# pyani-plus/pyani-plus

Measured on AMD Instinct MI355X. Metric: pairwise genome comparisons/sec (N x N ANI matrix), higher is better.
Workload: dtype u64

## Files before the change

### pyani_plus_amd/csrc/kmer_hash.hip

```cpp
#include <cstdlib>
#include <type_traits>
#include <utility>

#include "pa_internal.h"
#include "murmur_dev.h"

namespace {

using namespace pa_dev;

constexpr int kThreads = 256;
constexpr uint32_t kStageCap = 1024;
constexpr uint32_t kStageCapSecond = 512;

constexpr int pow2_floor(int k) { int c = 1; while (2 * c <= k) c *= 2; return c; }

__device__ __forceinline__ uint32_t find_genome(const uint32_t *__restrict__ genome_blk, uint32_t n, uint32_t blk) {
  uint32_t lo = 0, hi = n;
  while (hi - lo > 1) {
    uint32_t mid = (lo + hi) >> 1;
    if (genome_blk[mid] <= blk) lo = mid; else hi = mid;
  }
  return lo;
}
// ... 26 lines not shown
    region_append(s, find_genome(s.genome_blk, s.n_genomes, t), h);
  } else {
    const unsigned long long g = atomicAdd(reinterpret_cast<unsigned long long *>(s.count), 1ULL);
    if (g < s.cap) {
      s.cand_hash[g] = h;
      s.cand_genome[g] = find_genome(s.genome_blk, s.n_genomes, t);
    }
  }
}

template <uint32_t Cap>
__device__ __forceinline__ void flush_staged(const CandSink &s, const uint64_t (&s_hash)[Cap], const uint32_t (&s_blk)[Cap],
                                             const uint32_t &s_n, unsigned long long &s_base, uint32_t blk0, uint32_t n_blocks64) {
  const uint32_t tid = threadIdx.x;
  __syncthreads();
  const uint32_t n = min(s_n, Cap);
  if (n == 0) return;
  if (s.region_off) {
    const uint32_t b0 = blk0 + blockIdx.x * kThreads;
    const uint32_t b1 = min(b0 + (uint32_t)kThreads, n_blocks64) - 1u;
    const uint32_t g0 = find_genome(s.genome_blk, s.n_genomes, b0);
    if (s.genome_blk[g0 + 1] > b1) {
      if (tid == 0) s_base = atomicAdd(&s.cursor[g0], n);
      __syncthreads();
      const uint64_t room = s.region_off[g0 + 1] - s.region_off[g0];
      uint64_t *__restrict__ dst = s.cand_hash + s.region_off[g0];
      for (uint32_t i = tid; i < n; i += kThreads) {
        const uint64_t slot = s_base + i;
        if (slot < room) dst[slot] = s_hash[i]; else *s.overflow = 1u;
      }
    } else {
      for (uint32_t i = tid; i < n; i += kThreads)
        region_append(s, find_genome(s.genome_blk, s.n_genomes, s_blk[i]), s_hash[i]);
    }
    return;
  }
  if (tid == 0) s_base = atomicAdd(reinterpret_cast<unsigned long long *>(s.count), (unsigned long long)n);
  __syncthreads();
  const unsigned long long base = s_base;
  for (uint32_t i = tid; i < n; i += kThreads) {
    const unsigned long long g = base + i;
    if (g < s.cap) {
      s.cand_hash[g] = s_hash[i];
      s.cand_genome[g] = find_genome(s.genome_blk, s.n_genomes, s_blk[i]);
    }
  }
}

__device__ __forceinline__ uint32_t rev_groups32(uint32_t x) {
  x = __builtin_bitreverse32(x);
  return ((x >> 1) & 0x55555555u) | ((x & 0x55555555u) << 1);
}

enum WordForm { kArithmetic = 0, kFirstTables = 1, kSecondTables = 2 };
template <int K, WordForm FORM>
__global__ __launch_bounds__(kThreads) void kmer_hash_kernel(
    const uint4 *__restrict__ packed, const uint2 *__restrict__ mask, const uint64_t *__restrict__ dirty, uint32_t n_blocks64,
    const uint32_t *__restrict__ genome_blk, uint32_t n_genomes, uint64_t max_hash,
    uint64_t *__restrict__ cand_hash, uint32_t *__restrict__ cand_genome, uint64_t cap,
    unsigned long long *__restrict__ count, const uint64_t *__restrict__ region_off, uint32_t *__restrict__ cursor,
    uint32_t *__restrict__ overflow, uint32_t blk0) {
  static_assert(K >= 1 && K <= 32, "a k-mer is one 64-bit register pair");
  constexpr uint32_t kCap = FORM == kSecondTables ? kStageCapSecond : kStageCap;
  __shared__ uint64_t s_hash[kCap];
  __shared__ uint32_t s_blk[kCap];
  __shared__ uint32_t s_n;
  __shared__ unsigned long long s_base;
  constexpr int kWords = (K + 7) / 8;
  __shared__ uint64_t s_lo[FORM == kFirstTables ? kWords : 1][256];
  __shared__ uint4 s_w[FORM == kSecondTables ? kWords : 1][256];
  __shared__ uint32_t s_hi[FORM != kArithmetic ? kWords : 1][256];

  const uint32_t tid = threadIdx.x;
  const CandSink sink{cand_hash, cand_genome, cap, reinterpret_cast<uint64_t *>(count), region_off, cursor, overflow, genome_blk, n_genomes};
  const uint32_t max_hi = (uint32_t)(max_hash >> 32);
  const bool take_all = max_hi == 0xffffffffu;
  const uint32_t screen_hi = max_hi + 1u;
  if (tid == 0) s_n = 0;
  if constexpr (FORM == kFirstTables) fill_first_products(s_lo, s_hi, tid, std::integral_constant<int, K>{});
  if constexpr (FORM == kSecondTables) fill_second_products(s_w, s_hi, tid, K);
  __syncthreads();

  const uint32_t t = blk0 + blockIdx.x * kThreads + tid;
  if (t < n_blocks64) {
    const uint4 cur = packed[t];
    uint2 pw = make_uint2(0u, 0u);
    if (t > 0) pw = reinterpret_cast<const uint2 *>(packed)[2 * (uint64_t)t - 1];
    uint32_t d1 = 0u, d2 = 0u;
    const uint32_t wave_blk = __builtin_amdgcn_readfirstlane(t & ~63u);
    const uint64_t dirty_word = dirty[wave_blk >> 6];
    if ((dirty_word >> (t & 63u)) & 1ull) {
      const uint2 m = mask[t];
      uint32_t d0 = t > 0 ? mask[t - 1].y : 0xffffffffu;
      d1 = m.x;
      d2 = m.y;
      int c = 1;
#pragma unroll
      for (; 2 * c <= K; c *= 2) {
        d2 |= alignbit(d2, d1, 32 - c);
        d1 |= alignbit(d1, d0, 32 - c);
        d0 |= d0 << c;
      }
      constexpr int cc = pow2_floor(K);
      constexpr int r = K - cc;
      if constexpr (r > 0) {
        d2 |= alignbit(d2, d1, 32 - r);
        d1 |= alignbit(d1, d0, 32 - r);
      }
    }
    const uint32_t bad[2] = {d1, d2};
    if ((d1 & d2) != 0xffffffffu) {
      constexpr uint64_t kMask = (K == 32) ? ~0ULL : ((1ULL << (2 * K)) - 1);
      constexpr uint32_t kMaskHi = (uint32_t)(kMask >> 32);
      uint32_t fw[8] = {pw.x, pw.y, cur.x, cur.y, cur.z, cur.w, 0u, 0u};
      uint32_t rw[6];
#pragma unroll
      for (int j = 0; j < 6; ++j) rw[j] = ~rev_groups32(fw[5 - j]);
      auto columns = [&](auto base_tag, int i_begin, int i_end) {
        constexpr int kBase = decltype(base_tag)::value;
#pragma unroll 1
        for (int i = i_begin; i < i_end; ++i) {
          constexpr int kOff = 33 - K;
          const uint32_t fo = 2u * (uint32_t)((i + kOff) & 15), ro = 30u - 2u * (uint32_t)i;
          uint32_t A[5], B[5];
#pragma unroll
          for (int j = 0; j < 5; ++j) {
            A[j] = alignbit(fw[kBase + j + 1], fw[kBase + j], fo);
            B[j] = alignbit(rw[j + 1], rw[j], ro);
          }
#pragma unroll
          for (int wi = 0; wi < 4; ++wi) {
            const uint32_t f_lo = A[wi], f_hi = A[wi + 1], r_lo = B[3 - wi], r_hi = B[4 - wi];
          const uint64_t f_lsb = u64_of(f_lo, f_hi) & kMask, r_lsb = u64_of(r_lo, r_hi) & kMask;
          const uint64_t fwd = __builtin_amdgcn_uicmpl(f_lsb, r_lsb, 37 );
          uint32_t clo, chi;
          asm("s_nop 1\n\tv_cndmask_b32_e64 %0, %1, %2, %3" : "=v"(clo) : "v"((uint32_t)r_lsb), "v"((uint32_t)f_lsb), "s"(fwd));
          asm("v_cndmask_b32_e64 %0, %1, %2, %3" : "=v"(chi) : "v"((uint32_t)(r_lsb >> 32)), "v"((uint32_t)(f_lsb >> 32)), "s"(fwd), "v"(clo));
          uint64_t P[4] = {0, 0, 0, 0};
#pragma unroll
          for (int j = 0; j < kWords; ++j) {
            const uint32_t src = j < 2 ? clo : chi;
            if constexpr (FORM == kSecondTables) {
              P[j] = second_product(s_w, s_hi, j, src);
            } else if constexpr (FORM == kFirstTables) {
              P[j] = first_product(s_lo, s_hi, j, src);
            } else {
              const uint32_t glo = (src >> (16 * (j & 1))) & 0xffu, ghi = (src >> (16 * (j & 1) + 8)) & 0xffu;
              const uint64_t word = u64_of(ascii_group(glo, K - 8 * j), ascii_group(ghi, K - 8 * j - 4));
              P[j] = word * ((j & 1) ? kC2 : kC1);
            }
          }
          (void)kMaskHi;
          uint64_t U, V;
          if constexpr (FORM == kSecondTables) murmur3_pre_last_mul_of_seconds<K>(P, U, V); else murmur3_pre_last_mul<K>(P, U, V);
          if (passes_screen(U, V, take_all, screen_hi)) {
            const uint64_t h = last_mul_and_fold(U, V);
            if (h > max_hash || ((bad[wi >> 1] >> (16 * (wi & 1) + i)) & 1u)) continue;
            stage_candidate(sink, s_hash, s_blk, s_n, t, h);
          }
          }
        }
      };
      constexpr int kOff0 = 33 - K, kSplit = (kOff0 & 15) ? 16 - (kOff0 & 15) : 16;
      columns(std::integral_constant<int, (kOff0 >> 4)>{}, 0, kSplit);
      if constexpr (kSplit < 16) columns(std::integral_constant<int, (kOff0 >> 4) + 1>{}, kSplit, 16);
    }
  }
  flush_staged(sink, s_hash, s_blk, s_n, s_base, blk0, n_blocks64);
}

template <int K>
__global__ __launch_bounds__(kThreads) void kmer_hash_wide_kernel(
    const uint4 *__restrict__ packed, const uint2 *__restrict__ mask, const uint64_t *__restrict__ dirty, uint32_t n_blocks64,
    const uint32_t *__restrict__ genome_blk, uint32_t n_genomes, uint64_t max_hash,
    uint64_t *__restrict__ cand_hash, uint32_t *__restrict__ cand_genome, uint64_t cap,
    unsigned long long *__restrict__ count, const uint64_t *__restrict__ region_off, uint32_t *__restrict__ cursor,
    uint32_t *__restrict__ overflow, uint32_t blk0) {
  static_assert(K >= 33 && K <= 64, "k-mers of 65 to 128 bits");
  __shared__ uint64_t s_hash[kStageCap];
  __shared__ uint32_t s_blk[kStageCap];
  __shared__ uint32_t s_n;
  __shared__ unsigned long long s_base;
  constexpr int kWords = (K + 7) / 8;
  __shared__ uint64_t s_lo[kWords][256];
  __shared__ uint32_t s_hi[kWords][256];
  const uint32_t tid = threadIdx.x;
  const CandSink sink{cand_hash, cand_genome, cap, reinterpret_cast<uint64_t *>(count), region_off, cursor, overflow, genome_blk, n_genomes};
  const uint32_t max_hi = (uint32_t)(max_hash >> 32);
  const bool take_all = max_hi == 0xffffffffu;
  const uint32_t screen_hi = max_hi + 1u;
  if (tid == 0) s_n = 0;
  fill_first_products(s_lo, s_hi, tid, std::integral_constant<int, K>{});
  __syncthreads();

  const uint32_t t = blk0 + blockIdx.x * kThreads + tid;
  if (t < n_blocks64) {
    const uint4 cur = packed[t];
    const uint4 prev = t > 0 ? packed[t - 1] : make_uint4(0u, 0u, 0u, 0u);
    uint32_t d2 = 0u, d3 = 0u;
    const uint32_t wave_blk = __builtin_amdgcn_readfirstlane(t & ~63u);
    const uint64_t dirty_word = dirty[wave_blk >> 6];
    const uint64_t before = wave_blk ? dirty[(wave_blk >> 6) - 1] >> 63 : 1ull;
    const uint64_t dirty_or_prev = dirty_word | (dirty_word << 1) | before;
    if ((dirty_or_prev >> (t & 63u)) & 1ull) {
      const uint2 m = mask[t];
      uint32_t d0 = 0xffffffffu, d1 = 0xffffffffu;
      if (t > 0) { const uint2 mp = mask[t - 1]; d0 = mp.x; d1 = mp.y; }
      d2 = m.x;
// ... 88 lines not shown
  const uint64_t wg_first = pos0 + ((uint64_t)blockIdx.y * gridDim.x + blockIdx.x) * (uint64_t)(kThreads * kLongIter);
#pragma unroll 1
  for (int it = 0; it < kLongIter; ++it) {
  const uint64_t e = wg_first + (uint64_t)it * kThreads + tid;
  if (e >= pos1 || e + 1 < k) continue;
  const uint64_t a = e + 1 - k;
  {
    const uint64_t m0 = a >> 5, m_last = e >> 5;
    const uint32_t sm = (uint32_t)(a & 31u);
    const uint32_t w0 = mask[m0], w1 = m0 + 1 <= m_last ? mask[m0 + 1] : 0u, w2 = m0 + 2 <= m_last ? mask[m0 + 2] : 0u;
    const uint32_t b0 = alignbit(w1, w0, sm), b1 = alignbit(w2, w1, sm);
    const uint32_t top = k == 64 ? 0xffffffffu : ((1u << (k - 32u)) - 1u);
    if (b0 | (b1 & top)) continue;
  }
  uint32_t F[4], R[4];
  {
    const uint64_t p0 = a >> 4, p_last = e >> 4;
    const uint32_t sp = 2u * (uint32_t)(a & 15u);
    uint32_t w[5];
#pragma unroll
    for (int i = 0; i < 5; ++i) w[i] = p0 + i <= p_last ? packed[p0 + i] : 0u;
#pragma unroll
    for (int i = 0; i < 4; ++i) F[i] = alignbit(w[i + 1], w[i], sp);
    const uint32_t used = 2u * k - 64u;
    if (used < 32u) { F[2] &= (1u << used) - 1u; F[3] = 0u; }
    else if (used < 64u) F[3] &= (1u << (used - 32u)) - 1u;
    const uint32_t C[6] = {~rev_groups32(F[3]), ~rev_groups32(F[2]), ~rev_groups32(F[1]), ~rev_groups32(F[0]), 0u, 0u};
    const uint32_t s = 128u - 2u * k, ws = s >> 5, bs = s & 31u;
#pragma unroll
    for (int i = 0; i < 4; ++i) R[i] = ws ? alignbit(C[i + 2], C[i + 1], bs) : alignbit(C[i + 1], C[i], bs);
    if (used < 32u) { R[2] &= (1u << used) - 1u; R[3] = 0u; }
    else if (used < 64u) R[3] &= (1u << (used - 32u)) - 1u;
  }
  const uint64_t f_hi = u64_of(F[2], F[3]), f_lo = u64_of(F[0], F[1]), r_hi = u64_of(R[2], R[3]), r_lo = u64_of(R[0], R[1]);
  const bool fwd = f_hi < r_hi || (f_hi == r_hi && f_lo <= r_lo);
  uint32_t c[4];
#pragma unroll
  for (int i = 0; i < 4; ++i) c[i] = fwd ? F[i] : R[i];
  uint64_t P[8] = {0, 0, 0, 0, 0, 0, 0, 0};
#pragma unroll
  for (uint32_t j = 0; j < 8; ++j) {
    if (j >= n_words) break;
    P[j] = first_product(s_lo, s_hi, j, c[j >> 1]);
  }
  uint64_t U, V;
  murmur3_pre_last_mul_rt(P, k, U, V);
  if (!passes_screen(U, V, take_all, screen_hi)) continue;
  const uint64_t h = last_mul_and_fold(U, V);
  if (h > max_hash) continue;
  append_candidate(sink, find_genome(genome_blk, n_genomes, (uint32_t)(e >> 6)), h);
  }
}

template <class Kernel>
int launch_blocks(pa_ctx *c, const char *name, Kernel kernel, const KmerHashArgs &a) {
  const ArenaView &v = a.arena;
  const CandSink &s = a.sink;
  return pa_launch(c, name, kernel, false, ceil_div(v.n_blocks64 - a.blk0, kThreads), kThreads, 0, a.stream,
                   reinterpret_cast<const uint4 *>(v.packed), reinterpret_cast<const uint2 *>(v.mask), v.dirty,
                   (uint32_t)v.n_blocks64, s.genome_blk, s.n_genomes, a.max_hash, s.cand_hash, s.cand_genome, s.cap,
                   reinterpret_cast<unsigned long long *>(s.count), s.region_off, s.cursor, s.overflow, (uint32_t)a.blk0);
}

template <int K>
int launch_k(pa_ctx *c, const KmerHashArgs &a) {
  if constexpr (K > 32) {
    return launch_blocks(c, "kmer_hash_wide_kernel", kmer_hash_wide_kernel<K>, a);
  } else {
#ifdef PA_TOOLS
    if constexpr (K == 31) {
      const char *v = PA_TOOL_ENV("PA_KMER_VARIANT");
      if (v && v[0] == '0') return launch_blocks(c, "kmer_hash_kernel<31, kArithmetic>", kmer_hash_kernel<K, kArithmetic>, a);
      if (v && v[0] == '1') return launch_blocks(c, "kmer_hash_kernel<31, kFirstTables>", kmer_hash_kernel<K, kFirstTables>, a);
    }
#endif
    return launch_blocks(c, "kmer_hash_kernel", kmer_hash_kernel<K, kSecondTables>, a);
  }
}

}

int pa_launch_kmer_hash(pa_ctx *c, const KmerHashArgs &a) {
  const uint64_t n_blocks64 = a.arena.n_blocks64;
  PA_REQUIRE(n_blocks64 < (1ULL << 32), "arena too large: %llu blocks of 64 bases", (unsigned long long)n_blocks64);
  if (n_blocks64 <= a.blk0) return PA_OK;
  const char *long_form = PA_TOOL_ENV("PA_KMER_LONG");
  if (a.k > 32 && a.k <= 64 && long_form && long_form[0] == 'p') {
    const CandSink &s = a.sink;
    const uint64_t pos0 = a.blk0 * 64, pos1 = n_blocks64 * 64;
    const uint64_t per_wg = (uint64_t)kThreads * kLongIter;
    const uint64_t n_wg = (pos1 - pos0 + per_wg - 1) / per_wg;
    const uint32_t gx = (uint32_t)std::min<uint64_t>(n_wg, 1u << 20), gy = (uint32_t)((n_wg + gx - 1) / gx);
    PA_REQUIRE(gy <= 65535u, "arena too large for one launch of the long k-mer kernel: %llu positions", (unsigned long long)(pos1 - pos0));
    return PA_LAUNCH_ON(c, a.stream, kmer_hash_long_kernel, LaunchDim(gx, gy), kThreads, 0, a.arena.packed, a.arena.mask, pos0, pos1, a.k,
                        s.genome_blk, s.n_genomes, a.max_hash, s.cand_hash, s.cand_genome, s.cap,
                        reinterpret_cast<unsigned long long *>(s.count), s.region_off, s.cursor, s.overflow);
  }
  PA_REQUIRE((a.blk0 & 63u) == 0, "k-mer hash launch must start at a multiple of 64 blocks, not %llu", (unsigned long long)a.blk0);
  int status = PA_E_INVALID;
  if (!dispatch_value(a.k, value_list<1, 64>{}, [&](auto k) { status = launch_k<k()>(c, a); })) pa_set_error("k=%u outside [1,64]", a.k);
  return status;
}
```

### pyani_plus_amd/csrc/murmur_dev.h

```cpp
#pragma once

#include <hip/hip_runtime.h>

#include <cstdint>

#include "murmur_words.h"

namespace pa_dev {

__device__ __forceinline__ uint32_t alignbit(uint32_t hi, uint32_t lo, uint32_t sh) {
  return __builtin_amdgcn_alignbit(hi, lo, sh);
}

__device__ __forceinline__ uint64_t u64_of(uint32_t lo, uint32_t hi) { return ((uint64_t)hi << 32) | lo; }

__device__ __forceinline__ uint64_t rotl64(uint64_t x, int r) {
  const uint32_t lo = (uint32_t)x, hi = (uint32_t)(x >> 32);
  if (r == 32) return u64_of(hi, lo);
  if (r < 32) return u64_of(alignbit(lo, hi, 32 - r), alignbit(hi, lo, 32 - r));
  return u64_of(alignbit(hi, lo, 64 - r), alignbit(lo, hi, 64 - r));
}

__device__ __forceinline__ uint64_t fmix64(uint64_t k) {
  k ^= k >> 33;
  k *= 0xff51afd7ed558ccdULL;
  k ^= k >> 33;
  k *= 0xc4ceb9fe1a85ec53ULL;
  k ^= k >> 33;
  return k;
}


__device__ __forceinline__ uint64_t times5_plus(uint64_t h, uint64_t c) {
  uint64_t t;
  asm("v_lshl_add_u64 %0, %1, 2, %1" : "=v"(t) : "v"(h));
  return t + c;
}

constexpr uint64_t kF1 = 0xff51afd7ed558ccdULL, kF2 = 0xc4ceb9fe1a85ec53ULL;

template <int K, int N>
__device__ __forceinline__ void murmur3_pre_last_mul(const uint64_t (&P)[N], uint64_t &U, uint64_t &V) {
  static_assert(N >= (K + 7) / 8, "one first product per 8-byte word of the k-mer");
  uint64_t h1 = 42, h2 = 42;
  constexpr int nblocks = K / 16;
  constexpr int tail = K % 16;
#pragma unroll
  for (int i = 0; i < nblocks; ++i) {
    const uint64_t k1 = rotl64(P[2 * i], 31) * kC2;
    h1 ^= k1;
    if (i == 0) {
      h1 = times5_plus(rotl64(h1, 27), 5ULL * 42ULL + 0x52dce729ULL);
    } else {
      h1 = rotl64(h1, 27) + h2;
      h1 = times5_plus(h1, 0x52dce729ULL);
    }
    const uint64_t k2 = rotl64(P[2 * i + 1], 33) * kC1;
    h2 ^= k2;
    h2 = rotl64(h2, 31) + h1;
    h2 = times5_plus(h2, 0x38495ab5ULL);
  }
  if constexpr (tail > 8) h2 ^= rotl64(P[2 * nblocks + 1], 33) * kC1;
  if constexpr (tail > 0) h1 ^= rotl64(P[2 * nblocks], 31) * kC2;
  h1 ^= (uint64_t)K; h2 ^= (uint64_t)K;
  h1 += h2; h2 += h1;
  h1 ^= h1 >> 33; h1 *= kF1; h1 ^= h1 >> 33;
  h2 ^= h2 >> 33; h2 *= kF1; h2 ^= h2 >> 33;
  U = h1;
  V = h2;
}

template <int K, int N>
__device__ __forceinline__ void murmur3_pre_last_mul_of_seconds(const uint64_t (&Kw)[N], uint64_t &U, uint64_t &V) {
  static_assert(N >= (K + 7) / 8, "one second product per 8-byte word of the k-mer");
  uint64_t h1 = 42, h2 = 42;
  constexpr int nblocks = K / 16;
  constexpr int tail = K % 16;
#pragma unroll
  for (int i = 0; i < nblocks; ++i) {
    h1 ^= Kw[2 * i];
    if (i == 0) {
      h1 = times5_plus(rotl64(h1, 27), 5ULL * 42ULL + 0x52dce729ULL);
    } else {
      h1 = rotl64(h1, 27) + h2;
      h1 = times5_plus(h1, 0x52dce729ULL);
    }
    h2 ^= Kw[2 * i + 1];
    uint64_t r2 = rotl64(h2, 31);
    asm("" : "+v"(r2));
    h2 = times5_plus(r2 + h1, 0x38495ab5ULL);
  }
  if constexpr (tail > 8) h2 ^= Kw[2 * nblocks + 1];
  if constexpr (tail > 0) h1 ^= Kw[2 * nblocks];
  h1 ^= (uint64_t)K; h2 ^= (uint64_t)K;
  h1 += h2; h2 += h1;
  h1 ^= h1 >> 33; h1 *= kF1; h1 ^= h1 >> 33;
  h2 ^= h2 >> 33; h2 *= kF1; h2 ^= h2 >> 33;
  U = h1;
  V = h2;
}

__device__ __forceinline__ void murmur3_pre_last_mul_rt(const uint64_t (&P)[8], uint32_t k, uint64_t &U, uint64_t &V) {
  uint64_t h1 = 42, h2 = 42;
  const uint32_t nblocks = k >> 4, tail = k & 15u;
#pragma unroll
  for (uint32_t i = 0; i < 4; ++i) {
    if (i >= nblocks) break;
    h1 ^= rotl64(P[2 * i], 31) * kC2;
    h1 = rotl64(h1, 27) + h2;
    h1 = times5_plus(h1, 0x52dce729ULL);
    h2 ^= rotl64(P[2 * i + 1], 33) * kC1;
    h2 = rotl64(h2, 31) + h1;
    h2 = times5_plus(h2, 0x38495ab5ULL);
  }
  uint64_t t1 = 0, t2 = 0;
#pragma unroll
  for (uint32_t i = 0; i < 4; ++i)
    if (i == nblocks) { t1 = P[2 * i]; t2 = P[2 * i + 1]; }
  if (tail > 8) h2 ^= rotl64(t2, 33) * kC1;
  if (tail > 0) h1 ^= rotl64(t1, 31) * kC2;
  h1 ^= (uint64_t)k;
  h2 ^= (uint64_t)k;
  h1 += h2;
  h2 += h1;
  h1 ^= h1 >> 33; h1 *= kF1; h1 ^= h1 >> 33;
  h2 ^= h2 >> 33; h2 *= kF1; h2 ^= h2 >> 33;
  U = h1;
  V = h2;
}

__device__ __forceinline__ uint32_t last_mul_high_sum_plus1(uint64_t U, uint64_t V) {
  constexpr uint32_t c0 = (uint32_t)kF2, c1 = (uint32_t)(kF2 >> 32);
  const uint32_t u0 = (uint32_t)U, u1 = (uint32_t)(U >> 32), v0 = (uint32_t)V, v1 = (uint32_t)(V >> 32);
  return (__umulhi(u0, c0) + __umulhi(v0, c0) + 1u) + ((u0 + v0) * c1 + (u1 + v1) * c0);
}

__device__ __forceinline__ bool passes_screen(uint64_t U, uint64_t V, bool take_all, uint32_t screen_hi) {
  return take_all || last_mul_high_sum_plus1(U, V) <= screen_hi;
}
__device__ __forceinline__ uint64_t last_mul_and_fold(uint64_t U, uint64_t V) {
  const uint64_t X = U * kF2, Y = V * kF2;
  return (X ^ (X >> 33)) + (Y ^ (Y >> 33));
}

template <int K, int N>
__device__ __forceinline__ uint64_t murmur3_from_products(const uint64_t (&P)[N]) {
  uint64_t U, V;
  murmur3_pre_last_mul<K, N>(P, U, V);
  return last_mul_and_fold(U, V);
}

template <int W, class KInt>
__device__ __forceinline__ void fill_first_products(uint64_t (&s_lo)[W][256], uint32_t (&s_hi)[W][256], uint32_t tid, KInt k_) {
  const int k = (int)k_;
  const int n_words = (int)(((uint32_t)k + 7u) >> 3);
#pragma unroll
  for (int j = 0; j < n_words; ++j) {
    const uint64_t cj = (j & 1) ? kC2 : kC1;
    s_lo[j][tid] = (uint64_t)ascii_group(tid, k - 8 * j) * cj;
    s_hi[j][tid] = (uint32_t)((uint64_t)ascii_group(tid, k - 8 * j - 4) * cj);
  }
}

template <int W>
__device__ __forceinline__ uint64_t first_product(const uint64_t (&s_lo)[W][256], const uint32_t (&s_hi)[W][256], uint32_t j, uint32_t src) {
  const uint32_t glo = (src >> (16u * (j & 1u))) & 0xffu, ghi = (src >> (16u * (j & 1u) + 8u)) & 0xffu;
  const uint64_t lo = s_lo[j][glo];
  return u64_of((uint32_t)lo, (uint32_t)(lo >> 32) + s_hi[j][ghi]);
}

template <int W>
__device__ __forceinline__ void fill_second_products(uint4 (&s_w)[W][256], uint32_t (&s_b)[W][256], uint32_t tid, int k) {
#pragma unroll
  for (int j = 0; j < W; ++j) {
    const WordLoEntry e = word_lo_entry(j, k, tid);
    s_w[j][tid] = make_uint4(e.t_lo, e.t_hi, e.a_hi, e.pad);
    s_b[j][tid] = word_hi_entry(j, k, tid);
  }
}

template <uint32_t SH>
__device__ __forceinline__ uint32_t byte_offset(uint32_t src, uint32_t byte) {
  uint32_t r;
  const uint32_t sh = SH;
  switch (byte) {
    case 0: asm("v_lshlrev_b32_sdwa %0, %1, %2 dst_sel:DWORD dst_unused:UNUSED_PAD src0_sel:DWORD src1_sel:BYTE_0" : "=v"(r) : "v"(sh), "v"(src)); break;
    case 1: asm("v_lshlrev_b32_sdwa %0, %1, %2 dst_sel:DWORD dst_unused:UNUSED_PAD src0_sel:DWORD src1_sel:BYTE_1" : "=v"(r) : "v"(sh), "v"(src)); break;
    case 2: asm("v_lshlrev_b32_sdwa %0, %1, %2 dst_sel:DWORD dst_unused:UNUSED_PAD src0_sel:DWORD src1_sel:BYTE_2" : "=v"(r) : "v"(sh), "v"(src)); break;
    default: asm("v_lshlrev_b32_sdwa %0, %1, %2 dst_sel:DWORD dst_unused:UNUSED_PAD src0_sel:DWORD src1_sel:BYTE_3" : "=v"(r) : "v"(sh), "v"(src)); break;
  }
  return r;
}

template <int W>
__device__ __forceinline__ uint64_t second_product(const uint4 (&s_w)[W][256], const uint32_t (&s_b)[W][256], int j, uint32_t src) {
  const uint32_t off_w = byte_offset<4>(src, 2u * (j & 1)), off_b = byte_offset<2>(src, 2u * (j & 1) + 1u);
  typedef uint32_t u32x4 __attribute__((ext_vector_type(4)));
  u32x4 e = *reinterpret_cast<const u32x4 *>(reinterpret_cast<const char *>(&s_w[j][0]) + off_w);
  asm("" : "+v"(e));
  const uint32_t b = *reinterpret_cast<const uint32_t *>(reinterpret_cast<const char *>(&s_b[j][0]) + off_b);
  return second_product_of(j, e.x, e.y, e.z, b);
}

}
```

### pyani_plus_amd/csrc/murmur_words.h

```cpp
#pragma once

#include <cstdint>

#if defined(__HIPCC__)
#include <hip/hip_runtime.h>
#define PA_WORDS_FN __host__ __device__ __forceinline__
#else
#define PA_WORDS_FN inline
#endif

namespace pa_dev {

constexpr uint64_t kC1 = 0x87c37b91114253d5ULL, kC2 = 0x4cf5ad432745937fULL;

PA_WORDS_FN uint32_t ascii4(uint32_t b8) {
#if defined(__HIP_DEVICE_COMPILE__)
  uint32_t u = (b8 | (b8 << 12)) & 0x000F000Fu;
  uint32_t v = (u | (u << 6)) & 0x03030303u;
  return __builtin_amdgcn_perm(0u, 0x54474341u, v);
#else
  uint32_t a = 0;
  for (int i = 0; i < 4; ++i) a |= ((0x54474341u >> (8 * ((b8 >> (2 * i)) & 3u))) & 0xffu) << (8 * i);
  return a;
#endif
}

PA_WORDS_FN uint32_t ascii_group(uint32_t b8, int nv) {
  const uint32_t a = ascii4(b8);
  return nv >= 4 ? a : (nv <= 0 ? 0u : (a & ((1u << (8 * nv)) - 1u)));
}

PA_WORDS_FN constexpr uint64_t word_c_first(int j) { return (j & 1) ? kC2 : kC1; }
PA_WORDS_FN constexpr uint64_t word_c_second(int j) { return (j & 1) ? kC1 : kC2; }

struct WordLoEntry {
  uint32_t t_lo, t_hi, a_hi, pad;
};

PA_WORDS_FN WordLoEntry word_lo_entry(int j, int k, uint32_t g) {
  const uint64_t a = (uint64_t)ascii_group(g, k - 8 * j) * word_c_first(j);
  const uint32_t a_lo = (uint32_t)a;
  const uint64_t cb = word_c_second(j);
  const uint64_t t = (j & 1) ? (((uint64_t)a_lo << 33) + (a_lo >> 31)) * cb : ((uint64_t)a_lo << 31) * cb;
  return WordLoEntry{(uint32_t)t, (uint32_t)(t >> 32), (uint32_t)(a >> 32), 0u};
}

PA_WORDS_FN uint32_t word_hi_entry(int j, int k, uint32_t g) {
  return (uint32_t)((uint64_t)ascii_group(g, k - 8 * j - 4) * word_c_first(j));
}

PA_WORDS_FN uint64_t second_product_of(int j, uint32_t t_lo, uint32_t t_hi, uint32_t a_hi, uint32_t b) {
  const uint32_t s = a_hi + b;
  const uint64_t t = ((uint64_t)t_hi << 32) | t_lo;
  if (j & 1) {
    const uint64_t c = word_c_second(j) << 1;
    const uint64_t m = (uint64_t)s * (uint32_t)c + t;
    return ((uint64_t)((uint32_t)(m >> 32) + s * (uint32_t)(c >> 32)) << 32) | (uint32_t)m;
  }
  const uint64_t c = word_c_second(j);
  const uint32_t x = s >> 1;
  const uint64_t m = (uint64_t)x * (uint32_t)c + t;
  return ((uint64_t)((uint32_t)(m >> 32) + (x * (uint32_t)(c >> 32) + (s << 31))) << 32) | (uint32_t)m;
}

}
```

### pyani_plus_amd/csrc/pa_internal.h

```cpp
#pragma once

#include <hip/hip_runtime.h>

#include <algorithm>
#include <cstdarg>
#include <cstdint>
#include <cstdio>
#include <cstring>
#include <initializer_list>
#include <string>
#include <type_traits>
#include <vector>

#include "../../include/pyani_hip.h"
#include "pa_launch_geom.h"

void pa_set_error(const char *fmt, ...);

#define PA_HIP(call)                                                                          \
  do {                                                                                        \
    hipError_t _e = (call);                                                                   \
    if (_e != hipSuccess) {                                                                   \
      pa_set_error("%s failed: %s (%s:%d)", #call, hipGetErrorString(_e), __FILE__, __LINE__); \
      return PA_E_HIP;                                                                        \
// ... 63 lines not shown
  void release() {
    if (p) (void)hipFree(p);
    if (budget) budget->held -= bytes;
    p = nullptr;
    bytes = 0;
  }
  template <typename T>
  T *as() const { return reinterpret_cast<T *>(p); }
};

struct ProfPhase {
  double total_ms = 0.0;
  uint64_t launches = 0;
  std::vector<std::pair<hipEvent_t, hipEvent_t>> pending;
};

struct ScalarSlot {
  uint32_t word, words;
  constexpr uint32_t bytes() const { return words * 4u; }
  constexpr bool apart_from(ScalarSlot o) const { return word + words <= o.word || o.word + o.words <= word; }
};
constexpr bool slots_apart(uint32_t region_bytes, std::initializer_list<ScalarSlot> slots) {
  for (const ScalarSlot *a = slots.begin(); a != slots.end(); ++a) {
    if ((a->word + a->words) * 4u > region_bytes || (a->words % 2 == 0 && a->word % 2)) return false;
    for (const ScalarSlot *b = a + 1; b != slots.end(); ++b)
      if (!a->apart_from(*b)) return false;
  }
  return true;
}

constexpr uint32_t kCtxScalarBytes = 128;
constexpr ScalarSlot kCandCount{0, 2};
constexpr ScalarSlot kSketchTotal{2, 2};
constexpr ScalarSlot kDenseIds{4, 4};
constexpr uint32_t kDenseOr = 0, kDenseDistinct = 1;
constexpr ScalarSlot kCompactTotal{8, 2};
constexpr ScalarSlot kRegionOverflow{12, 1};
constexpr ScalarSlot kNjPick{16, 8};
constexpr ScalarSlot kNjBad{24, 4};
static_assert(slots_apart(kCtxScalarBytes, {kCandCount, kSketchTotal, kDenseIds, kCompactTotal, kRegionOverflow, kNjPick, kNjBad}),
              "two slots of pa_ctx::counters overlap or leave the block");

constexpr uint32_t kDictScalarBytes = 64;
constexpr ScalarSlot kDictCounters{0, 2};
constexpr uint32_t kDictIdCounter = 0, kDictSpecialId = 1;
constexpr ScalarSlot kDictPreparedFp{2, 4};
constexpr ScalarSlot kDictTileFp{6, 4};
static_assert(slots_apart(kDictScalarBytes, {kDictCounters, kDictPreparedFp, kDictTileFp}),
              "two slots of pa_ctx::dict_scalars overlap or leave the block");

constexpr uint32_t kPinnedBytes = 64;

#define PA_CTX_BUFFERS(ONE, PAIR)                                                                                   \
  PAIR(cand_keys) PAIR(cand_vals) ONE(genome_blk) ONE(counters) ONE(hist) ONE(flags) ONE(scan_tmp) ONE(region_off) \
  ONE(region_cursor) ONE(dirty) PAIR(dict_keys) PAIR(dict_vals) ONE(ids) ONE(post_genome) ONE(bitrows)             \
  ONE(dict_scalars) ONE(cls_i) ONE(cls_j) ONE(cls_score) ONE(cls_cov) ONE(bin2d) ONE(tetra_tab) ONE(nj_work)

struct pa_ctx {
  int device = 0;
  hipStream_t stream = nullptr;
  bool own_stream = false;
  hipDeviceProp_t prop;
#define PA_ONE(name) DevBuf name;
#define PA_PAIR(name) DevBuf name[2];
  PA_CTX_BUFFERS(PA_ONE, PA_PAIR)
#undef PA_ONE
#undef PA_PAIR
  template <class Fn>
  void each_buffer(Fn &&fn) {
#define PA_ONE(name) fn(name);
#define PA_PAIR(name) fn(name[0]); fn(name[1]);
    PA_CTX_BUFFERS(PA_ONE, PA_PAIR)
#undef PA_ONE
#undef PA_PAIR
  }
  template <typename T = uint32_t>
  T *slot(ScalarSlot s) const { return reinterpret_cast<T *>(counters.as<uint32_t>() + s.word); }
  template <typename T = uint32_t>
  T *dict_slot(ScalarSlot s) const { return reinterpret_cast<T *>(dict_scalars.as<uint32_t>() + s.word); }
  bool dict_prepared = false;
  uint64_t dict_prepared_postings = 0;
  uint32_t dict_prepared_cap = 0;
  hipStream_t copy_stream = nullptr;
  void *frag_work = nullptr;
  uint64_t *h_pinned = nullptr;
  bool prof_on = false;
  ProfPhase prof[PA_PROF_NPHASES];
  std::vector<hipEvent_t> event_pool;
};

class ReadBack {
 public:
  explicit ReadBack(pa_ctx *c) : c_(c) {}
  template <typename T>
  int queue(const T *d_src, T *out, uint32_t count = 1) {
    static_assert(std::is_trivially_copyable<T>::value && alignof(T) <= 8, "ReadBack copies plain scalars");
    const uint64_t bytes = (uint64_t)count * sizeof(T);
    PA_REQUIRE(n_ < kMaxItems && used_ + bytes <= kPinnedBytes, "read-back of %llu bytes behind %u in %u copies exceeds the pinned block of %u bytes",
               (unsigned long long)bytes, used_, n_, kPinnedBytes);
    PA_HIP(hipMemcpyAsync(reinterpret_cast<char *>(c_->h_pinned) + used_, d_src, bytes, hipMemcpyDeviceToHost, c_->stream));
    items_[n_++] = Item{out, used_, (uint32_t)bytes};
    used_ = (used_ + (uint32_t)bytes + 7u) & ~7u;
    return PA_OK;
  }
  int wait() {
    PA_HIP(hipStreamSynchronize(c_->stream));
    for (uint32_t i = 0; i < n_; ++i) memcpy(items_[i].out, reinterpret_cast<const char *>(c_->h_pinned) + items_[i].at, items_[i].bytes);
    n_ = used_ = 0;
    return PA_OK;
  }

 private:
  static constexpr uint32_t kMaxItems = 4;
  struct Item {
    void *out;
    uint32_t at, bytes;
  };
  pa_ctx *c_;
  Item items_[kMaxItems];
  uint32_t n_ = 0, used_ = 0;
};
template <typename T>
int pa_read_back(pa_ctx *c, const T *d_src, T *out, uint32_t count = 1) {
  ReadBack rb(c);
  PA_TRY(rb.queue(d_src, out, count));
  return rb.wait();
}

struct ProfScope {
  pa_ctx *c;
  int phase;
  hipEvent_t e0 = nullptr, e1 = nullptr;
  ProfScope(pa_ctx *ctx, int ph);
  ~ProfScope();
};
// ... 139 lines not shown
```

Before: 81.88 million.

## Precompute k-mer hash lookup tables on host and copy them into shared memory

Each block now copies per-k lookup tables from a device image instead of computing the second-product tables itself. The image is built once per k on the host, cached on the device, and deduplicates words whose table contents match. This shrinks shared memory use, which may raise occupancy, and removes per-block table arithmetic. The candidate screen also switches to a sum-based screen word with a slightly looser bound, which may let a few more candidates reach the exact check.

```diff
diff --git a/pyani_plus_amd/csrc/kmer_hash.hip b/pyani_plus_amd/csrc/kmer_hash.hip
--- a/pyani_plus_amd/csrc/kmer_hash.hip
+++ b/pyani_plus_amd/csrc/kmer_hash.hip
@@ -109,7 +109,7 @@
     const uint32_t *__restrict__ genome_blk, uint32_t n_genomes, uint64_t max_hash,
     uint64_t *__restrict__ cand_hash, uint32_t *__restrict__ cand_genome, uint64_t cap,
     unsigned long long *__restrict__ count, const uint64_t *__restrict__ region_off, uint32_t *__restrict__ cursor,
-    uint32_t *__restrict__ overflow, uint32_t blk0) {
+    uint32_t *__restrict__ overflow, uint32_t blk0, const uint4 *__restrict__ image) {
   static_assert(K >= 1 && K <= 32, "a k-mer is one 64-bit register pair");
   constexpr uint32_t kCap = FORM == kSecondTables ? kStageCapSecond : kStageCap;
   __shared__ uint64_t s_hash[kCap];
@@ -118,17 +118,20 @@
   __shared__ unsigned long long s_base;
   constexpr int kWords = (K + 7) / 8;
   __shared__ uint64_t s_lo[FORM == kFirstTables ? kWords : 1][256];
-  __shared__ uint4 s_w[FORM == kSecondTables ? kWords : 1][256];
-  __shared__ uint32_t s_hi[FORM != kArithmetic ? kWords : 1][256];
+  __shared__ uint32_t s_hi[FORM == kFirstTables ? kWords : 1][256];
+  __shared__ __attribute__((aligned(16))) unsigned char s_img[FORM == kSecondTables ? image_bytes(K) : 16];
 
   const uint32_t tid = threadIdx.x;
   const CandSink sink{cand_hash, cand_genome, cap, reinterpret_cast<uint64_t *>(count), region_off, cursor, overflow, genome_blk, n_genomes};
   const uint32_t max_hi = (uint32_t)(max_hash >> 32);
-  const bool take_all = max_hi == 0xffffffffu;
-  const uint32_t screen_hi = max_hi + 1u;
+  constexpr bool kSumScreen = FORM == kSecondTables;
+  const bool take_all = kSumScreen ? screen_takes_all(max_hi) : max_hi == 0xffffffffu;
+  const uint32_t screen_hi = max_hi + (kSumScreen ? 2u : 1u);
+  uint64_t screen_one_hi = 1ULL << 32;
+  asm("" : "+v"(screen_one_hi));
   if (tid == 0) s_n = 0;
   if constexpr (FORM == kFirstTables) fill_first_products(s_lo, s_hi, tid, std::integral_constant<int, K>{});
-  if constexpr (FORM == kSecondTables) fill_second_products(s_w, s_hi, tid, K);
+  if constexpr (FORM == kSecondTables) copy_image<K>(s_img, image, tid);
   __syncthreads();
 
   const uint32_t t = blk0 + blockIdx.x * kThreads + tid;
@@ -191,7 +194,7 @@
           for (int j = 0; j < kWords; ++j) {
             const uint32_t src = j < 2 ? clo : chi;
             if constexpr (FORM == kSecondTables) {
-              P[j] = second_product(s_w, s_hi, j, src);
+              P[j] = second_product<K>(s_img, j, src);
             } else if constexpr (FORM == kFirstTables) {
               P[j] = first_product(s_lo, s_hi, j, src);
             } else {
@@ -203,7 +206,7 @@
           (void)kMaskHi;
           uint64_t U, V;
           if constexpr (FORM == kSecondTables) murmur3_pre_last_mul_of_seconds<K>(P, U, V); else murmur3_pre_last_mul<K>(P, U, V);
-          if (passes_screen(U, V, take_all, screen_hi)) {
+          if (kSumScreen ? (take_all || screen_word(U, V, screen_one_hi) <= screen_hi) : passes_screen(U, V, take_all, screen_hi)) {
             const uint64_t h = last_mul_and_fold(U, V);
             if (h > max_hash || ((bad[wi >> 1] >> (16 * (wi & 1) + i)) & 1u)) continue;
             stage_candidate(sink, s_hash, s_blk, s_n, t, h);
@@ -398,14 +401,30 @@
   }
 }
 
-template <class Kernel>
-int launch_blocks(pa_ctx *c, const char *name, Kernel kernel, const KmerHashArgs &a) {
+template <class Kernel, class... Extra>
+int launch_blocks(pa_ctx *c, const char *name, Kernel kernel, const KmerHashArgs &a, Extra... extra) {
   const ArenaView &v = a.arena;
   const CandSink &s = a.sink;
   return pa_launch(c, name, kernel, false, ceil_div(v.n_blocks64 - a.blk0, kThreads), kThreads, 0, a.stream,
                    reinterpret_cast<const uint4 *>(v.packed), reinterpret_cast<const uint2 *>(v.mask), v.dirty,
                    (uint32_t)v.n_blocks64, s.genome_blk, s.n_genomes, a.max_hash, s.cand_hash, s.cand_genome, s.cap,
-                   reinterpret_cast<unsigned long long *>(s.count), s.region_off, s.cursor, s.overflow, (uint32_t)a.blk0);
+                   reinterpret_cast<unsigned long long *>(s.count), s.region_off, s.cursor, s.overflow, (uint32_t)a.blk0, extra...);
+}
+
+constexpr uint64_t kImageSlotBytes = (kImageMaxBytes + 255u) & ~255u;
+int image_on_device(pa_ctx *c, uint32_t k, hipStream_t stream, const uint4 **image) {
+  static_assert(sizeof(c->kmer_image_ready) / sizeof(c->kmer_image_ready[0]) == kImageMaxK + 1, "one flag per k");
+  PA_TRY(c->kmer_images.reserve((kImageMaxK + 1) * kImageSlotBytes));
+  unsigned char *slot = c->kmer_images.as<unsigned char>() + k * kImageSlotBytes;
+  if (!c->kmer_image_ready[k]) {
+    std::vector<unsigned char> host(image_bytes((int)k));
+    fill_image((int)k, host.data());
+    PA_HIP(hipMemcpyAsync(slot, host.data(), host.size(), hipMemcpyHostToDevice, stream ? stream : c->stream));
+    PA_HIP(hipStreamSynchronize(stream ? stream : c->stream));
+    c->kmer_image_ready[k] = true;
+  }
+  *image = reinterpret_cast<const uint4 *>(slot);
+  return PA_OK;
 }
 
 template <int K>
@@ -416,11 +435,14 @@
 #ifdef PA_TOOLS
     if constexpr (K == 31) {
       const char *v = PA_TOOL_ENV("PA_KMER_VARIANT");
-      if (v && v[0] == '0') return launch_blocks(c, "kmer_hash_kernel<31, kArithmetic>", kmer_hash_kernel<K, kArithmetic>, a);
-      if (v && v[0] == '1') return launch_blocks(c, "kmer_hash_kernel<31, kFirstTables>", kmer_hash_kernel<K, kFirstTables>, a);
+      const uint4 *none = nullptr;
+      if (v && v[0] == '0') return launch_blocks(c, "kmer_hash_kernel<31, kArithmetic>", kmer_hash_kernel<K, kArithmetic>, a, none);
+      if (v && v[0] == '1') return launch_blocks(c, "kmer_hash_kernel<31, kFirstTables>", kmer_hash_kernel<K, kFirstTables>, a, none);
     }
 #endif
-    return launch_blocks(c, "kmer_hash_kernel", kmer_hash_kernel<K, kSecondTables>, a);
+    const uint4 *image = nullptr;
+    PA_TRY(image_on_device(c, K, a.stream, &image));
+    return launch_blocks(c, "kmer_hash_kernel", kmer_hash_kernel<K, kSecondTables>, a, image);
   }
 }
 
diff --git a/pyani_plus_amd/csrc/murmur_dev.h b/pyani_plus_amd/csrc/murmur_dev.h
--- a/pyani_plus_amd/csrc/murmur_dev.h
+++ b/pyani_plus_amd/csrc/murmur_dev.h
@@ -36,8 +36,6 @@
   asm("v_lshl_add_u64 %0, %1, 2, %1" : "=v"(t) : "v"(h));
   return t + c;
 }
-
-constexpr uint64_t kF1 = 0xff51afd7ed558ccdULL, kF2 = 0xc4ceb9fe1a85ec53ULL;
 
 template <int K, int N>
 __device__ __forceinline__ void murmur3_pre_last_mul(const uint64_t (&P)[N], uint64_t &U, uint64_t &V) {
@@ -169,14 +167,13 @@
   return u64_of((uint32_t)lo, (uint32_t)(lo >> 32) + s_hi[j][ghi]);
 }
 
-template <int W>
-__device__ __forceinline__ void fill_second_products(uint4 (&s_w)[W][256], uint32_t (&s_b)[W][256], uint32_t tid, int k) {
-#pragma unroll
-  for (int j = 0; j < W; ++j) {
-    const WordLoEntry e = word_lo_entry(j, k, tid);
-    s_w[j][tid] = make_uint4(e.t_lo, e.t_hi, e.a_hi, e.pad);
-    s_b[j][tid] = word_hi_entry(j, k, tid);
-  }
+template <int K>
+__device__ __forceinline__ void copy_image(unsigned char *s_img, const uint4 *__restrict__ image, uint32_t tid) {
+  constexpr uint32_t n16 = image_bytes(K) / 16u;
+  uint4 *dst = reinterpret_cast<uint4 *>(s_img);
+#pragma unroll
+  for (uint32_t i = 0; i < n16; i += 256u)
+    if (i + 256u <= n16 || i + tid < n16) dst[i + tid] = image[i + tid];
 }
 
 template <uint32_t SH>
@@ -192,13 +189,14 @@
   return r;
 }
 
-template <int W>
-__device__ __forceinline__ uint64_t second_product(const uint4 (&s_w)[W][256], const uint32_t (&s_b)[W][256], int j, uint32_t src) {
-  const uint32_t off_w = byte_offset<4>(src, 2u * (j & 1)), off_b = byte_offset<2>(src, 2u * (j & 1) + 1u);
+template <int K>
+__device__ __forceinline__ uint64_t second_product(const unsigned char *s_img, int j, uint32_t src) {
+  const uint32_t off_w = byte_offset<4>(src, 2u * (j & 1));
   typedef uint32_t u32x4 __attribute__((ext_vector_type(4)));
-  u32x4 e = *reinterpret_cast<const u32x4 *>(reinterpret_cast<const char *>(&s_w[j][0]) + off_w);
+  u32x4 e = *reinterpret_cast<const u32x4 *>(&s_img[image_lo_offset(j, K)] + off_w);
   asm("" : "+v"(e));
-  const uint32_t b = *reinterpret_cast<const uint32_t *>(reinterpret_cast<const char *>(&s_b[j][0]) + off_b);
+  uint32_t b = 0u;
+  if (image_has_hi(j, K)) b = *reinterpret_cast<const uint32_t *>(&s_img[image_hi_offset(j, K)] + byte_offset<2>(src, 2u * (j & 1) + 1u));
   return second_product_of(j, e.x, e.y, e.z, b);
 }
 
diff --git a/pyani_plus_amd/csrc/murmur_words.h b/pyani_plus_amd/csrc/murmur_words.h
--- a/pyani_plus_amd/csrc/murmur_words.h
+++ b/pyani_plus_amd/csrc/murmur_words.h
@@ -63,4 +63,70 @@
   return ((uint64_t)((uint32_t)(m >> 32) + (x * (uint32_t)(c >> 32) + (s << 31))) << 32) | (uint32_t)m;
 }
 
+
+constexpr uint32_t kImageLoTableBytes = 256u * 16u;
+PA_WORDS_FN constexpr int image_words(int k) { return (k + 7) / 8; }
+PA_WORDS_FN constexpr int word_lo_bases(int j, int k) { return k - 8 * j < 4 ? k - 8 * j : 4; }
+PA_WORDS_FN constexpr int word_hi_bases(int j, int k) { return k - 8 * j - 4 < 0 ? 0 : (k - 8 * j - 4 < 4 ? k - 8 * j - 4 : 4); }
+constexpr uint32_t kImageHiTableBytes = 256u * 4u;
+
+PA_WORDS_FN constexpr int image_lo_class(int j, int k) {
+  for (int i = j & 1; i < j; i += 2)
+    if (word_lo_bases(i, k) == word_lo_bases(j, k)) return i;
+  return j;
 }
+PA_WORDS_FN constexpr int image_hi_class(int j, int k) {
+  for (int i = j & 1; i < j; i += 2)
+    if (word_hi_bases(i, k) == word_hi_bases(j, k)) return i;
+  return j;
+}
+PA_WORDS_FN constexpr bool image_has_hi(int j, int k) { return word_hi_bases(j, k) > 0; }
+
+PA_WORDS_FN constexpr uint32_t image_lo_offset(int j, int k) {
+  uint32_t off = 0;
+  for (int i = 0; i < image_lo_class(j, k); ++i)
+    if (image_lo_class(i, k) == i) off += kImageLoTableBytes;
+  return off;
+}
+PA_WORDS_FN constexpr uint32_t image_lo_bytes(int k) {
+  uint32_t off = 0;
+  for (int i = 0; i < image_words(k); ++i)
+    if (image_lo_class(i, k) == i) off += kImageLoTableBytes;
+  return off;
+}
+PA_WORDS_FN constexpr uint32_t image_hi_offset(int j, int k) {
+  uint32_t off = image_lo_bytes(k);
+  for (int i = 0; i < image_hi_class(j, k); ++i)
+    if (image_has_hi(i, k) && image_hi_class(i, k) == i) off += kImageHiTableBytes;
+  return off;
+}
+PA_WORDS_FN constexpr uint32_t image_bytes(int k) {
+  uint32_t off = image_lo_bytes(k);
+  for (int i = 0; i < image_words(k); ++i)
+    if (image_has_hi(i, k) && image_hi_class(i, k) == i) off += kImageHiTableBytes;
+  return off;
+}
+constexpr int kImageMaxK = 32;
+constexpr uint32_t kImageMaxBytes = 4u * (kImageLoTableBytes + kImageHiTableBytes);
+
+inline void fill_image(int k, unsigned char *out) {
+  for (int j = 0; j < image_words(k); ++j) {
+    if (image_lo_class(j, k) == j) {
+      WordLoEntry *lo = reinterpret_cast<WordLoEntry *>(out + image_lo_offset(j, k));
+      for (uint32_t g = 0; g < 256; ++g) lo[g] = word_lo_entry(j, k, g);
+    }
+    if (image_has_hi(j, k) && image_hi_class(j, k) == j) {
+      uint32_t *hi = reinterpret_cast<uint32_t *>(out + image_hi_offset(j, k));
+      for (uint32_t g = 0; g < 256; ++g) hi[g] = word_hi_entry(j, k, g);
+    }
+  }
+}
+
+constexpr uint64_t kF1 = 0xff51afd7ed558ccdULL, kF2 = 0xc4ceb9fe1a85ec53ULL;
+PA_WORDS_FN constexpr bool screen_takes_all(uint32_t max_hi) { return max_hi >= 0xfffffffeu; }
+PA_WORDS_FN uint32_t screen_word(uint64_t U, uint64_t V, uint64_t one_hi = 1ULL << 32) { return (uint32_t)(((U + V) * kF2 + one_hi) >> 32); }
+PA_WORDS_FN bool passes_sum_screen(uint64_t U, uint64_t V, uint32_t max_hi) {
+  return screen_takes_all(max_hi) || screen_word(U, V) <= max_hi + 2u;
+}
+
+}
diff --git a/pyani_plus_amd/csrc/pa_internal.h b/pyani_plus_amd/csrc/pa_internal.h
--- a/pyani_plus_amd/csrc/pa_internal.h
+++ b/pyani_plus_amd/csrc/pa_internal.h
@@ -139,8 +139,8 @@
 constexpr uint32_t kPinnedBytes = 64;
 
 #define PA_CTX_BUFFERS(ONE, PAIR)                                                                                   \
-  PAIR(cand_keys) PAIR(cand_vals) ONE(genome_blk) ONE(counters) ONE(hist) ONE(flags) ONE(scan_tmp) ONE(region_off) \
-  ONE(region_cursor) ONE(dirty) PAIR(dict_keys) PAIR(dict_vals) ONE(ids) ONE(post_genome) ONE(bitrows)             \
+  PAIR(cand_keys) PAIR(cand_vals) ONE(genome_blk) ONE(kmer_images) ONE(counters) ONE(hist) ONE(flags) ONE(scan_tmp) \
+  ONE(region_off) ONE(region_cursor) ONE(dirty) PAIR(dict_keys) PAIR(dict_vals) ONE(ids) ONE(post_genome) ONE(bitrows) \
   ONE(dict_scalars) ONE(cls_i) ONE(cls_j) ONE(cls_score) ONE(cls_cov) ONE(bin2d) ONE(tetra_tab) ONE(nj_work)
 
 struct pa_ctx {
@@ -168,6 +168,7 @@
   bool dict_prepared = false;
   uint64_t dict_prepared_postings = 0;
   uint32_t dict_prepared_cap = 0;
+  bool kmer_image_ready[33] = {};
   hipStream_t copy_stream = nullptr;
   void *frag_work = nullptr;
   uint64_t *h_pinned = nullptr;
```

Measured after the change: 84.25 million (median of 6 runs). 2.9% higher.

## Share second-product tables by word role and screen candidates on summed product

Applied to the files above, without the earlier changes.

Word tables in shared memory are now keyed by role (parity plus number of valid bases), so words with identical roles share one table slot and empty high groups skip their LDS load. The candidate screen now computes one high-half product of U+V instead of separate products, using a looser bound. The odd-word hi computation uses a fused shift-add instruction. This aims to cut LDS footprint, loads and ALU work in the hot per-k-mer path, at the cost of a looser screen that may let more candidates through to the full hash.

```diff
diff --git a/pyani_plus_amd/csrc/kmer_hash.hip b/pyani_plus_amd/csrc/kmer_hash.hip
--- a/pyani_plus_amd/csrc/kmer_hash.hip
+++ b/pyani_plus_amd/csrc/kmer_hash.hip
@@ -102,7 +102,7 @@
   return ((x >> 1) & 0x55555555u) | ((x & 0x55555555u) << 1);
 }
 
-enum WordForm { kArithmetic = 0, kFirstTables = 1, kSecondTables = 2 };
+enum WordForm { kArithmetic = 0, kFirstTables = 1, kSecondTables = 2, kSecondTablesPerWord = 3 };
 template <int K, WordForm FORM>
 __global__ __launch_bounds__(kThreads) void kmer_hash_kernel(
     const uint4 *__restrict__ packed, const uint2 *__restrict__ mask, const uint64_t *__restrict__ dirty, uint32_t n_blocks64,
@@ -111,24 +111,33 @@
     unsigned long long *__restrict__ count, const uint64_t *__restrict__ region_off, uint32_t *__restrict__ cursor,
     uint32_t *__restrict__ overflow, uint32_t blk0) {
   static_assert(K >= 1 && K <= 32, "a k-mer is one 64-bit register pair");
-  constexpr uint32_t kCap = FORM == kSecondTables ? kStageCapSecond : kStageCap;
+  constexpr bool kSeconds = FORM == kSecondTables || FORM == kSecondTablesPerWord;
+  constexpr bool kByRole = FORM == kSecondTables;
+  constexpr bool kSumScreen = FORM == kSecondTables;
+  constexpr bool kShiftAdd = FORM == kSecondTables;
+  using Tab = SecondTables<K, kByRole>;
+  constexpr uint32_t kCap = kSeconds ? kStageCapSecond : kStageCap;
   __shared__ uint64_t s_hash[kCap];
   __shared__ uint32_t s_blk[kCap];
   __shared__ uint32_t s_n;
   __shared__ unsigned long long s_base;
   constexpr int kWords = (K + 7) / 8;
   __shared__ uint64_t s_lo[FORM == kFirstTables ? kWords : 1][256];
-  __shared__ uint4 s_w[FORM == kSecondTables ? kWords : 1][256];
-  __shared__ uint32_t s_hi[FORM != kArithmetic ? kWords : 1][256];
+  __shared__ uint4 s_w[kSeconds ? Tab::kLoSlots : 1][256];
+  __shared__ uint32_t s_hi[kSeconds ? (Tab::kHiSlots > 0 ? Tab::kHiSlots : 1) : FORM == kFirstTables ? kWords : 1][256];
 
   const uint32_t tid = threadIdx.x;
   const CandSink sink{cand_hash, cand_genome, cap, reinterpret_cast<uint64_t *>(count), region_off, cursor, overflow, genome_blk, n_genomes};
   const uint32_t max_hi = (uint32_t)(max_hash >> 32);
   const bool take_all = max_hi == 0xffffffffu;
   const uint32_t screen_hi = max_hi + 1u;
+  const bool take_all_sum = screen_takes_all(max_hash);
+  const uint32_t screen_bound = screen_bound_of(max_hash);
+  uint64_t two32 = kTwo32;
+  if constexpr (FORM == kSecondTables) asm volatile("" : "+v"(two32));
   if (tid == 0) s_n = 0;
   if constexpr (FORM == kFirstTables) fill_first_products(s_lo, s_hi, tid, std::integral_constant<int, K>{});
-  if constexpr (FORM == kSecondTables) fill_second_products(s_w, s_hi, tid, K);
+  if constexpr (kSeconds) fill_second_products<K, kByRole>(s_w, s_hi, tid);
   __syncthreads();
 
   const uint32_t t = blk0 + blockIdx.x * kThreads + tid;
@@ -190,8 +199,8 @@
 #pragma unroll
           for (int j = 0; j < kWords; ++j) {
             const uint32_t src = j < 2 ? clo : chi;
-            if constexpr (FORM == kSecondTables) {
-              P[j] = second_product(s_w, s_hi, j, src);
+            if constexpr (kSeconds) {
+              P[j] = second_product<K, kByRole, kShiftAdd>(s_w, s_hi, j, src);
             } else if constexpr (FORM == kFirstTables) {
               P[j] = first_product(s_lo, s_hi, j, src);
             } else {
@@ -202,8 +211,8 @@
           }
           (void)kMaskHi;
           uint64_t U, V;
-          if constexpr (FORM == kSecondTables) murmur3_pre_last_mul_of_seconds<K>(P, U, V); else murmur3_pre_last_mul<K>(P, U, V);
-          if (passes_screen(U, V, take_all, screen_hi)) {
+          if constexpr (kSeconds) murmur3_pre_last_mul_of_seconds<K>(P, U, V); else murmur3_pre_last_mul<K>(P, U, V);
+          if (kSumScreen ? passes_screen_sum(U, V, take_all_sum, screen_bound, two32) : passes_screen(U, V, take_all, screen_hi)) {
             const uint64_t h = last_mul_and_fold(U, V);
             if (h > max_hash || ((bad[wi >> 1] >> (16 * (wi & 1) + i)) & 1u)) continue;
             stage_candidate(sink, s_hash, s_blk, s_n, t, h);
@@ -418,6 +427,7 @@
       const char *v = PA_TOOL_ENV("PA_KMER_VARIANT");
       if (v && v[0] == '0') return launch_blocks(c, "kmer_hash_kernel<31, kArithmetic>", kmer_hash_kernel<K, kArithmetic>, a);
       if (v && v[0] == '1') return launch_blocks(c, "kmer_hash_kernel<31, kFirstTables>", kmer_hash_kernel<K, kFirstTables>, a);
+      if (v && v[0] == '2') return launch_blocks(c, "kmer_hash_kernel<31, kSecondTablesPerWord>", kmer_hash_kernel<K, kSecondTablesPerWord>, a);
     }
 #endif
     return launch_blocks(c, "kmer_hash_kernel", kmer_hash_kernel<K, kSecondTables>, a);
diff --git a/pyani_plus_amd/csrc/murmur_dev.h b/pyani_plus_amd/csrc/murmur_dev.h
--- a/pyani_plus_amd/csrc/murmur_dev.h
+++ b/pyani_plus_amd/csrc/murmur_dev.h
@@ -36,8 +36,6 @@
   asm("v_lshl_add_u64 %0, %1, 2, %1" : "=v"(t) : "v"(h));
   return t + c;
 }
-
-constexpr uint64_t kF1 = 0xff51afd7ed558ccdULL, kF2 = 0xc4ceb9fe1a85ec53ULL;
 
 template <int K, int N>
 __device__ __forceinline__ void murmur3_pre_last_mul(const uint64_t (&P)[N], uint64_t &U, uint64_t &V) {
@@ -138,10 +136,6 @@
 __device__ __forceinline__ bool passes_screen(uint64_t U, uint64_t V, bool take_all, uint32_t screen_hi) {
   return take_all || last_mul_high_sum_plus1(U, V) <= screen_hi;
 }
-__device__ __forceinline__ uint64_t last_mul_and_fold(uint64_t U, uint64_t V) {
-  const uint64_t X = U * kF2, Y = V * kF2;
-  return (X ^ (X >> 33)) + (Y ^ (Y >> 33));
-}
 
 template <int K, int N>
 __device__ __forceinline__ uint64_t murmur3_from_products(const uint64_t (&P)[N]) {
@@ -169,13 +163,26 @@
   return u64_of((uint32_t)lo, (uint32_t)(lo >> 32) + s_hi[j][ghi]);
 }
 
-template <int W>
-__device__ __forceinline__ void fill_second_products(uint4 (&s_w)[W][256], uint32_t (&s_b)[W][256], uint32_t tid, int k) {
-#pragma unroll
-  for (int j = 0; j < W; ++j) {
-    const WordLoEntry e = word_lo_entry(j, k, tid);
-    s_w[j][tid] = make_uint4(e.t_lo, e.t_hi, e.a_hi, e.pad);
-    s_b[j][tid] = word_hi_entry(j, k, tid);
+template <int K, bool BY_ROLE>
+struct SecondTables {
+  static constexpr int kWords = word_count(K);
+  static constexpr int kLoSlots = BY_ROLE ? word_slot_count(K, false) : kWords;
+  static constexpr int kHiSlots = BY_ROLE ? word_slot_count(K, true) : kWords;
+  static constexpr bool fills(int j, bool hi) { return BY_ROLE ? word_fills_slot(j, K, hi) : true; }
+  static constexpr int slot(int j, bool hi) { return BY_ROLE ? word_slot(j, K, hi) : j; }
+};
+
+template <int K, bool BY_ROLE, int NW, int NB>
+__device__ __forceinline__ void fill_second_products(uint4 (&s_w)[NW][256], uint32_t (&s_b)[NB][256], uint32_t tid) {
+  using Tab = SecondTables<K, BY_ROLE>;
+  static_assert(NW >= Tab::kLoSlots && NB >= Tab::kHiSlots, "one table per slot");
+#pragma unroll
+  for (int j = 0; j < Tab::kWords; ++j) {
+    if (Tab::fills(j, false)) {
+      const WordLoEntry e = word_lo_entry(j, K, tid);
+      s_w[Tab::slot(j, false)][tid] = make_uint4(e.t_lo, e.t_hi, e.a_hi, e.pad);
+    }
+    if (Tab::fills(j, true)) s_b[Tab::slot(j, true)][tid] = word_hi_entry(j, K, tid);
   }
 }
 
@@ -192,14 +199,19 @@
   return r;
 }
 
-template <int W>
-__device__ __forceinline__ uint64_t second_product(const uint4 (&s_w)[W][256], const uint32_t (&s_b)[W][256], int j, uint32_t src) {
-  const uint32_t off_w = byte_offset<4>(src, 2u * (j & 1)), off_b = byte_offset<2>(src, 2u * (j & 1) + 1u);
+template <int K, bool BY_ROLE, bool SHIFT_ADD, int NW, int NB>
+__device__ __forceinline__ uint64_t second_product(const uint4 (&s_w)[NW][256], const uint32_t (&s_b)[NB][256], int j, uint32_t src) {
+  using Tab = SecondTables<K, BY_ROLE>;
+  const uint32_t off_w = byte_offset<4>(src, 2u * (j & 1));
   typedef uint32_t u32x4 __attribute__((ext_vector_type(4)));
-  u32x4 e = *reinterpret_cast<const u32x4 *>(reinterpret_cast<const char *>(&s_w[j][0]) + off_w);
+  u32x4 e = *reinterpret_cast<const u32x4 *>(reinterpret_cast<const char *>(&s_w[Tab::slot(j, false)][0]) + off_w);
   asm("" : "+v"(e));
-  const uint32_t b = *reinterpret_cast<const uint32_t *>(reinterpret_cast<const char *>(&s_b[j][0]) + off_b);
-  return second_product_of(j, e.x, e.y, e.z, b);
-}
-
-}
+  uint32_t b = 0u;
+  if (Tab::slot(j, true) >= 0) {
+    const uint32_t off_b = byte_offset<2>(src, 2u * (j & 1) + 1u);
+    b = *reinterpret_cast<const uint32_t *>(reinterpret_cast<const char *>(&s_b[Tab::slot(j, true)][0]) + off_b);
+  }
+  return second_product_of(j, e.x, e.y, e.z, b, SHIFT_ADD);
+}
+
+}
diff --git a/pyani_plus_amd/csrc/murmur_words.h b/pyani_plus_amd/csrc/murmur_words.h
--- a/pyani_plus_amd/csrc/murmur_words.h
+++ b/pyani_plus_amd/csrc/murmur_words.h
@@ -49,7 +49,7 @@
   return (uint32_t)((uint64_t)ascii_group(g, k - 8 * j - 4) * word_c_first(j));
 }
 
-PA_WORDS_FN uint64_t second_product_of(int j, uint32_t t_lo, uint32_t t_hi, uint32_t a_hi, uint32_t b) {
+PA_WORDS_FN uint64_t second_product_of(int j, uint32_t t_lo, uint32_t t_hi, uint32_t a_hi, uint32_t b, bool shift_add = false) {
   const uint32_t s = a_hi + b;
   const uint64_t t = ((uint64_t)t_hi << 32) | t_lo;
   if (j & 1) {
@@ -60,7 +60,67 @@
   const uint64_t c = word_c_second(j);
   const uint32_t x = s >> 1;
   const uint64_t m = (uint64_t)x * (uint32_t)c + t;
+#if defined(__HIP_DEVICE_COMPILE__)
+  if (shift_add) {
+    uint32_t hi;
+    asm("v_lshl_add_u32 %0, %1, 31, %2" : "=v"(hi) : "v"(s), "v"((uint32_t)(m >> 32)));
+    return ((uint64_t)(hi + x * (uint32_t)(c >> 32)) << 32) | (uint32_t)m;
+  }
+#endif
+  (void)shift_add;
   return ((uint64_t)((uint32_t)(m >> 32) + (x * (uint32_t)(c >> 32) + (s << 31))) << 32) | (uint32_t)m;
 }
 
+PA_WORDS_FN constexpr int word_count(int k) { return (k + 7) / 8; }
+PA_WORDS_FN constexpr int group_role(int parity, int n_valid) {
+  return n_valid <= 0 ? 0 : 1 + 4 * parity + ((n_valid < 4 ? n_valid : 4) - 1);
 }
+PA_WORDS_FN constexpr int word_lo_role(int j, int k) { return group_role(j & 1, k - 8 * j); }
+PA_WORDS_FN constexpr int word_hi_role(int j, int k) { return group_role(j & 1, k - 8 * j - 4); }
+PA_WORDS_FN constexpr int word_role(int j, int k, bool hi) { return hi ? word_hi_role(j, k) : word_lo_role(j, k); }
+
+PA_WORDS_FN constexpr bool word_fills_slot(int j, int k, bool hi) {
+  if (word_role(j, k, hi) == 0) return false;
+  for (int i = 0; i < j; ++i)
+    if (word_role(i, k, hi) == word_role(j, k, hi)) return false;
+  return true;
+}
+PA_WORDS_FN constexpr int word_slot(int j, int k, bool hi) {
+  if (word_role(j, k, hi) == 0) return -1;
+  int first = j;
+  for (int i = j - 1; i >= 0; --i)
+    if (word_role(i, k, hi) == word_role(j, k, hi)) first = i;
+  int slot = 0;
+  for (int i = 0; i < first; ++i) slot += word_fills_slot(i, k, hi) ? 1 : 0;
+  return slot;
+}
+PA_WORDS_FN constexpr int word_slot_count(int k, bool hi) {
+  int n = 0;
+  for (int j = 0; j < word_count(k); ++j) n += word_fills_slot(j, k, hi) ? 1 : 0;
+  return n;
+}
+
+constexpr uint64_t kF1 = 0xff51afd7ed558ccdULL, kF2 = 0xc4ceb9fe1a85ec53ULL;
+
+PA_WORDS_FN constexpr bool screen_takes_all(uint64_t max_hash) { return (uint32_t)(max_hash >> 32) >= 0xfffffffeu; }
+PA_WORDS_FN constexpr uint32_t screen_bound_of(uint64_t max_hash) { return (uint32_t)(max_hash >> 32) + 2u; }
+
+constexpr uint64_t kTwo32 = 1ULL << 32;
+PA_WORDS_FN uint32_t sum_product_high_plus1(uint64_t U, uint64_t V, uint64_t two32 = kTwo32) {
+  constexpr uint32_t c0 = (uint32_t)kF2, c1 = (uint32_t)(kF2 >> 32);
+  const uint64_t W = U + V;
+  const uint32_t w0 = (uint32_t)W, w1 = (uint32_t)(W >> 32);
+  const uint64_t m = (uint64_t)w0 * c0 + two32;
+  return (uint32_t)(m >> 32) + (w0 * c1 + w1 * c0);
+}
+
+PA_WORDS_FN bool passes_screen_sum(uint64_t U, uint64_t V, bool take_all, uint32_t screen_bound, uint64_t two32 = kTwo32) {
+  return take_all || sum_product_high_plus1(U, V, two32) <= screen_bound;
+}
+
+PA_WORDS_FN uint64_t last_mul_and_fold(uint64_t U, uint64_t V) {
+  const uint64_t X = U * kF2, Y = V * kF2;
+  return (X ^ (X >> 33)) + (Y ^ (Y >> 33));
+}
+
+}
```

Result: faster. 87.44 million before, 90.78 million after, median of 6 (+3.8%).
